# pjookim/srsran-ce-pytorch

Hardware: AMD Instinct MI355X
Metric: slots/sec (273-PRB PUSCH, 4 Rx) (higher is better)
Workload: dtype f32; 1 GPU; pusch273_4rx_filter; n_prb=273, n_sc=3276, n_sym=14, layers=1, rx_ports=4, smoothing=filter, interp=linear, slots_per_gpu=8192, global_slots=8192, rx_layout=[slot][port][sym][sc], parallelism=slot-shard x1, no collective

## Files before the change

srsran_ce_pytorch_amd/csrc/ce_denoise.hip:

```cpp
#include <hip/hip_runtime.h>
#include <stdint.h>
#include <string.h>

#include <type_traits>
#include <vector>

#include "ce_denoise.h"
#include "ce_plan.h"

typedef _Float16 half8 __attribute__((ext_vector_type(8)));
typedef _Float16 half4 __attribute__((ext_vector_type(4)));
typedef _Float16 half2v __attribute__((ext_vector_type(2)));
typedef float f32x4 __attribute__((ext_vector_type(4)));

struct ce_denoiser {
  int device = 0;
  half8* wfrag = nullptr;
  float* bias = nullptr;
};

#ifndef DN_ABLATE
#define DN_ABLATE 0
#endif

namespace {

#ifndef DN_MIN_WAVES
#define DN_MIN_WAVES 3
#endif
#ifndef DN_TWO_BODIES
#define DN_TWO_BODIES 0
#endif
#ifndef DN_L3_BUF
#define DN_L3_BUF 2
#endif
#ifndef DN_T_ROWS
#define DN_T_ROWS 32
#endif
constexpr int DN_T = DN_T_ROWS;
constexpr int DN_NB3 = DN_T / 16;
static_assert(DN_T % 16 == 0, "strip height");
constexpr int DN_NT = 256, DN_COLS = 16, DN_C = CE_DN_CHANNELS;
constexpr int X0_PIX = (DN_T + 6) * DN_COLS + 2;
constexpr int X1_PIX = (DN_T + 5) * DN_COLS + 2;
constexpr int X2_PIX = (DN_T + 2) * DN_COLS + 2;

__device__ __forceinline__ int tap_off(int tap) {
  const int ky = tap / 3, kx = tap - 3 * ky;
  return (ky - 1) * DN_COLS + (kx - 1);
}

constexpr int ROW_BYTES16 = DN_COLS * DN_C * 2;
constexpr int ROW_BYTES0 = DN_COLS * 4;

typedef _Float16 half2x __attribute__((ext_vector_type(2)));
__device__ __forceinline__ float2 masked(float2 v, bool ok) {
  const unsigned m = ok ? 0xFFFFFFFFu : 0u;
  return make_float2(__uint_as_float(__float_as_uint(v.x) & m), __uint_as_float(__float_as_uint(v.y) & m));
}
__device__ __forceinline__ half4 relu_h4(f32x4 acc, unsigned keep) {
  half2x lo = half2x{(_Float16)acc[0], (_Float16)acc[1]}, hi = half2x{(_Float16)acc[2], (_Float16)acc[3]};
  const half2x z = half2x{0, 0}, top = half2x{65504, 65504};
  lo = __builtin_elementwise_min(__builtin_elementwise_max(lo, z), top);
  hi = __builtin_elementwise_min(__builtin_elementwise_max(hi, z), top);
  unsigned ulo, uhi;
  __builtin_memcpy(&ulo, &lo, 4);
  __builtin_memcpy(&uhi, &hi, 4);
  ulo &= keep;
  uhi &= keep;
  __builtin_memcpy(&lo, &ulo, 4);
  __builtin_memcpy(&hi, &uhi, 4);
  return half4{lo[0], lo[1], hi[0], hi[1]};
}

__global__ __launch_bounds__(DN_NT, DN_MIN_WAVES) void ce_denoise_kernel(float2* __restrict__ ch, const half8* __restrict__ wfrag,
                                                            const float* __restrict__ bias, int n_sc, int L) {
  __shared__ __attribute__((aligned(16))) half2v x0[2][X0_PIX];
  __shared__ __attribute__((aligned(16))) _Float16 x1[X1_PIX * DN_C];
  __shared__ __attribute__((aligned(16))) _Float16 x2[X2_PIX * DN_C];
  const int tid = threadIdx.x, lane = tid & 63;
  const int wave = __builtin_amdgcn_readfirstlane(tid >> 6);
  const int n = lane & 15, g = lane >> 4;
  const int64_t plane = blockIdx.x;
  const int64_t item = plane / L;
  const int l = (int)(plane - item * L);
  float2* base = ch + item * (int64_t)n_sc * CE_DN_SYMBOLS * L + l;

  half8 w1 = wfrag[lane], w2[5], w3[9];
#pragma unroll
  for (int m = 0; m < 5; ++m) w2[m] = wfrag[(1 + m) * 64 + lane];
#pragma unroll
  for (int m = 0; m < 9; ++m) w3[m] = wfrag[(6 + m) * 64 + lane];
  f32x4 b1, b2, b3;
#pragma unroll
  for (int i = 0; i < 4; ++i) {
    b1[i] = bias[4 * g + i];
    b2[i] = bias[16 + 4 * g + i];
    b3[i] = g < 2 ? bias[32 + (i & 1)] : 0.f;
  }
  for (int i = tid; i < 2 * X0_PIX; i += DN_NT) (&x0[0][0])[i] = half2v{0, 0};
  for (int i = tid; i < X1_PIX * DN_C; i += DN_NT) x1[i] = 0;
  for (int i = tid; i < X2_PIX * DN_C; i += DN_NT) x2[i] = 0;

  const bool col_ok = n >= 1 && n <= CE_DN_SYMBOLS;
  const unsigned keep = col_ok ? 0xFFFFFFFFu : 0u;
  int rd0[4];
#pragma unroll
  for (int q = 0; q < 4; ++q) {
    const int tap = 4 * g + q;
    rd0[q] = (1 + (wave + 1) * DN_COLS + n + tap_off(tap < 9 ? tap : 4)) * 4;
  }
  constexpr int R2 = (DN_T + 2 + 3) / 4;
  const int a2 = wave * R2 < DN_T + 2 - R2 ? wave * R2 : DN_T + 2 - R2;
  int rdA, rdC, wr2;
  {
    const int pa = 1 + a2 * DN_COLS + n - 1 + (g >> 1), pc = 1 + (a2 + (g >> 1)) * DN_COLS + n + 1, pw = 1 + a2 * DN_COLS + n;
    rdA = pa * (DN_C * 2) + (((g & 1) ^ ((pa >> 2) & 1)) * 16);
    rdC = pc * (DN_C * 2) + (((g & 1) ^ ((pc >> 2) & 1)) * 16);
    wr2 = pw * (DN_C * 2) + ((((g >> 1) & 1) ^ ((pw >> 2) & 1)) * 16) + (g & 1) * 8;
  }
  const int wpix = 1 + wave * DN_COLS + n;
  const int wr = wpix * (DN_C * 2) + ((((g >> 1) & 1) ^ ((wpix >> 2) & 1)) * 16) + (g & 1) * 8;
  constexpr int ST_N = ((DN_T + 6) * DN_COLS + DN_NT - 1) / DN_NT;
  int st_off[ST_N], st_row[ST_N];
  bool st_ok[ST_N];
#pragma unroll
  for (int k = 0; k < ST_N; ++k) {
    const int i = tid + k * DN_NT, sym = (i & 15) - 1;
    st_row[k] = (i >> 4) - 3;
    st_ok[k] = i < (DN_T + 6) * DN_COLS && sym >= 0 && sym < CE_DN_SYMBOLS;
    st_off[k] = (st_row[k] * CE_DN_SYMBOLS + sym) * L;
  }
  int rd3[3];
#pragma unroll
  for (int dx = 0; dx < 3; ++dx) {
    const int pix = 1 + (4 * wave + 3 * (g >> 1)) * DN_COLS + n + dx - 1;
    rd3[dx] = pix * (DN_C * 2) + (((g & 1) ^ ((pix >> 2) & 1)) * 16);
  }
  const int h_row = 4 * wave + 2 * g;
  const int h_off = (h_row * CE_DN_SYMBOLS + (n - 1)) * L;
  const bool h_lane = g < 2 && col_ok;

  float2 st[ST_N];
  auto stage_load = [&](int r0) {
    const float2* sb = base + (int64_t)r0 * CE_DN_SYMBOLS * L;
#pragma unroll
    for (int k = 0; k < ST_N; ++k) {
      const bool ok = st_ok[k] && (unsigned)(r0 + st_row[k]) < (unsigned)n_sc;
      st[k] = masked((DN_ABLATE & 2) ? make_float2(0.f, 0.f) : sb[ok ? st_off[k] : 0], ok);
    }
  };
  auto stage_load_in = [&](int r0) {
    const float2* sb = base + (int64_t)r0 * CE_DN_SYMBOLS * L;
#pragma unroll
    for (int k = 0; k < ST_N; ++k) st[k] = masked((DN_ABLATE & 2) ? make_float2(0.f, 0.f) : sb[st_ok[k] ? st_off[k] : 0], st_ok[k]);
  };
  auto stage_store = [&](int buf) {
#pragma unroll
    for (int k = 0; k < ST_N; ++k) {
      const int i = tid + k * DN_NT;
      if (i < (DN_T + 6) * DN_COLS) x0[buf][1 + i] = half2v{(_Float16)st[k].x, (_Float16)st[k].y};
    }
  };
  stage_load(0);
  __syncthreads();
  stage_store(0);
  __syncthreads();
  const int n_strips = (n_sc + DN_T - 1) / DN_T;
  auto strip = [&](auto edge_tag, int s) __attribute__((always_inline)) {
    constexpr bool EDGE = decltype(edge_tag)::value;
    const int r0 = s * DN_T, buf = s & 1;
    float2* sb = base + (int64_t)r0 * CE_DN_SYMBOLS * L;
    if (s + 1 < n_strips) {
      if (!EDGE && r0 + 2 * DN_T + 3 <= n_sc) stage_load_in(r0 + DN_T); else stage_load(r0 + DN_T);
    }
    float2 hres[DN_NB3][2];
#pragma unroll
    for (int b = 0; b < DN_NB3; ++b)
#pragma unroll
      for (int e = 0; e < 2; ++e) {
        const bool ok = h_lane && (!EDGE || r0 + h_row + 16 * b + e < n_sc);
        hres[b][e] = masked((DN_ABLATE & 2) ? make_float2(0.f, 0.f) : sb[ok ? h_off + (16 * b + e) * CE_DN_SYMBOLS * L : 0], ok);
      }
    {
      const char* xin = reinterpret_cast<const char*>(&x0[buf][0]);
      char* xout = reinterpret_cast<char*>(x1);
      constexpr int NK1 = (DN_T + 4) / 4;
      auto finish1 = [&](f32x4 acc, int k) __attribute__((always_inline)) {
        const int row = r0 - 2 + wave + 4 * k;
        const unsigned rowkeep = (!EDGE || (row >= 0 && row < n_sc)) ? keep : 0u;
        *reinterpret_cast<half4*>(xout + wr + k * 4 * ROW_BYTES16) = relu_h4(acc, rowkeep);
      };
      f32x4 accp = b1;
      half2v px[2][4];
#pragma unroll
      for (int q = 0; q < 4; ++q) px[0][q] = *reinterpret_cast<const half2v*>(xin + rd0[q]);
#pragma unroll
      for (int k = 0; k < NK1; ++k) {
        if (k + 1 < NK1) {
#pragma unroll
          for (int q = 0; q < 4; ++q) px[(k + 1) & 1][q] = *reinterpret_cast<const half2v*>(xin + rd0[q] + (k + 1) * 4 * ROW_BYTES0);
        }
        asm volatile("" ::: "memory");
        half8 b;
#pragma unroll
        for (int q = 0; q < 4; ++q) {
          b[2 * q] = px[k & 1][q][0];
          b[2 * q + 1] = px[k & 1][q][1];
        }
        const f32x4 acc = __builtin_amdgcn_mfma_f32_16x16x32_f16(w1, b, b1, 0, 0, 0);
        if (k > 0) finish1(accp, k - 1);
        accp = acc;
      }
      finish1(accp, NK1 - 1);
    }
    __syncthreads();
    if (s + 1 < n_strips) stage_store(buf ^ 1);
    {
      const char* xin = reinterpret_cast<const char*>(x1);
      char* xout = reinterpret_cast<char*>(x2);
      half8 fa[R2 + 2], fc[R2 + 2];
      auto fetch = [&](int i) __attribute__((always_inline)) {
        fa[i] = *reinterpret_cast<const half8*>(xin + rdA + i * ROW_BYTES16);
        fc[i] = *reinterpret_cast<const half8*>(xin + rdC + i * ROW_BYTES16);
      };
      fetch(0);
      fetch(1);
      fetch(2);
      auto finish2 = [&](f32x4 acc, int j) __attribute__((always_inline)) {
        const int row = r0 - 1 + a2 + j;
        const unsigned rowkeep = (!EDGE || (row >= 0 && row < n_sc)) ? keep : 0u;
        *reinterpret_cast<half4*>(xout + wr2 + j * ROW_BYTES16) = relu_h4(acc, rowkeep);
      };
      f32x4 accp = b2;
#pragma unroll
      for (int j = 0; j < R2; ++j) {
        if (j + 3 < R2 + 2) fetch(j + 3);
        asm volatile("" ::: "memory");
        f32x4 acc = b2;
        acc = __builtin_amdgcn_mfma_f32_16x16x32_f16(w2[0], fa[j], acc, 0, 0, 0);
        acc = __builtin_amdgcn_mfma_f32_16x16x32_f16(w2[1], fa[j + 1], acc, 0, 0, 0);
        acc = __builtin_amdgcn_mfma_f32_16x16x32_f16(w2[2], fa[j + 2], acc, 0, 0, 0);
        acc = __builtin_amdgcn_mfma_f32_16x16x32_f16(w2[3], fc[j], acc, 0, 0, 0);
        acc = __builtin_amdgcn_mfma_f32_16x16x32_f16(w2[4], fc[j + 2], acc, 0, 0, 0);
        if (j > 0) finish2(accp, j - 1);
        accp = acc;
      }
      finish2(accp, R2 - 1);
    }
    __syncthreads();
    {
      const char* xin = reinterpret_cast<const char*>(x2);
      auto finish3 = [&](f32x4 acc, int b) __attribute__((always_inline)) {
#pragma unroll
        for (int e = 0; e < 2; ++e)
          if ((!(DN_ABLATE & 1) || acc[0] == 123.456f) && h_lane && (!EDGE || r0 + h_row + 16 * b + e < n_sc))
            sb[h_off + (16 * b + e) * CE_DN_SYMBOLS * L] = make_float2(hres[b][e].x + acc[2 * e], hres[b][e].y + acc[2 * e + 1]);
      };
      f32x4 accp = b3;
      half8 fr[DN_L3_BUF][9];
#pragma unroll
      for (int j = 0; j < 9; ++j) fr[0][j] = *reinterpret_cast<const half8*>(xin + rd3[j % 3] + (j / 3) * ROW_BYTES16);
#pragma unroll
      for (int b = 0; b < DN_NB3; ++b) {
        if (DN_L3_BUF == 2 && b + 1 < DN_NB3) {
#pragma unroll
          for (int j = 0; j < 9; ++j) fr[(b + 1) & 1][j] = *reinterpret_cast<const half8*>(xin + rd3[j % 3] + (16 * (b + 1) + j / 3) * ROW_BYTES16);
        }
        if (DN_L3_BUF == 1 && b > 0) {
#pragma unroll
          for (int j = 0; j < 9; ++j) fr[0][j] = *reinterpret_cast<const half8*>(xin + rd3[j % 3] + (16 * b + j / 3) * ROW_BYTES16);
        }
        asm volatile("" ::: "memory");
        f32x4 acc = b3;
#pragma unroll
        for (int j = 0; j < 9; ++j) acc = __builtin_amdgcn_mfma_f32_16x16x32_f16(w3[j], fr[b & (DN_L3_BUF - 1)][j], acc, 0, 0, 0);
        if (b > 0) finish3(accp, b - 1);
        accp = acc;
      }
      finish3(accp, DN_NB3 - 1);
    }
  };
#pragma unroll 1
  for (int s = 0; s < n_strips; ++s) {
    const int r0 = s * DN_T;
    if (DN_TWO_BODIES && r0 >= 3 && r0 + DN_T + 3 <= n_sc) strip(std::false_type{}, s);
    else strip(std::true_type{}, s);
  }
}

_Float16 to_h(float v) { return (_Float16)v; }

}

extern "C" int ce_denoiser_create(int32_t device, const float* w1, const float* b1, const float* w2, const float* b2,
                                  const float* w3, const float* b3, ce_denoiser** out) {
  if (!w1 || !b1 || !w2 || !b2 || !w3 || !b3 || !out) return ce_fail(CE_ERR_INVALID, "null argument");
  std::vector<_Float16> frag(15 * 64 * 8, to_h(0.f));
  auto at = [&](int f, int lane, int j) -> _Float16& { return frag[((size_t)f * 64 + lane) * 8 + j]; };
  for (int lane = 0; lane < 64; ++lane) {
    const int co = lane & 15, g = lane >> 4;
    for (int j = 0; j < 8; ++j) {
      const int k = 8 * g + j, tap = k >> 1, ci = k & 1;
      if (tap < 9) at(0, lane, j) = to_h(w1[(co * 2 + ci) * 9 + tap]);
    }
    for (int j = 0; j < 8; ++j) {
      const int ci = 8 * (g & 1) + j, up = g >> 1;
      for (int ky = 0; ky < 3; ++ky) at(1 + ky, lane, j) = to_h(w2[(co * 16 + ci) * 9 + ky * 3 + up]);
      at(4, lane, j) = to_h(w2[(co * 16 + ci) * 9 + up * 3 + 2]);
      if (!up) at(5, lane, j) = to_h(w2[(co * 16 + ci) * 9 + 2 * 3 + 2]);
    }
    if (co < 8)
      for (int m = 0; m < 9; ++m)
        for (int j = 0; j < 8; ++j) {
          const int r = co >> 1, c3 = co & 1, ri = m / 3 + 3 * (g >> 1), dx = m % 3, ci = 8 * (g & 1) + j, ky = ri - r;
          if (ky >= 0 && ky <= 2) at(6 + m, lane, j) = to_h(w3[(c3 * 16 + ci) * 9 + ky * 3 + dx]);
        }
  }
  float bias[48] = {0};
  for (int i = 0; i < 16; ++i) { bias[i] = b1[i]; bias[16 + i] = b2[i]; }
  bias[32] = b3[0];
  bias[33] = b3[1];
  ce_denoiser* d = new ce_denoiser;
  d->device = device;
  CeDeviceScope scope(device);
  hipError_t e = scope.err;
  if (e == hipSuccess) e = hipMalloc(&d->wfrag, frag.size() * sizeof(_Float16));
  if (e == hipSuccess) e = hipMalloc(&d->bias, sizeof(bias));
  if (e == hipSuccess) e = hipMemcpy(d->wfrag, frag.data(), frag.size() * sizeof(_Float16), hipMemcpyHostToDevice);
  if (e == hipSuccess) e = hipMemcpy(d->bias, bias, sizeof(bias), hipMemcpyHostToDevice);
  if (e != hipSuccess) {
    ce_denoiser_destroy(d);
    return ce_fail(CE_ERR_HIP, "denoiser upload: %s", hipGetErrorString(e));
  }
  *out = d;
  return CE_OK;
}

extern "C" void ce_denoiser_destroy(ce_denoiser* d) {
  if (!d) return;
  if (d->wfrag) (void)hipFree(d->wfrag);
  if (d->bias) (void)hipFree(d->bias);
  delete d;
}

extern "C" int ce_denoise_batch(const ce_denoiser* d, void* ch_est, int64_t n_items, int32_t n_sc, int32_t n_sym,
                                int32_t n_layers, void* stream) {
  if (!d || (!ch_est && n_items > 0)) return ce_fail(CE_ERR_INVALID, "null argument");
  if (n_sym != CE_DN_SYMBOLS) return ce_fail(CE_ERR_UNSUPPORTED, "the denoiser is built for 14-symbol grids (got %d)", n_sym);
  if (n_items < 0 || n_sc < 1 || n_layers < 1 || n_layers > CE_MAX_LAYERS) return ce_fail(CE_ERR_INVALID, "bad shape");
  const int64_t planes = n_items * n_layers;
  if (planes == 0) return CE_OK;
  if (planes > 0x7FFFFFFFll) return ce_fail(CE_ERR_UNSUPPORTED, "%lld planes in one launch", (long long)planes);
  CeDeviceScope scope(d->device);
  if (scope.err != hipSuccess) return ce_fail(CE_ERR_HIP, "device %d: %s", d->device, hipGetErrorString(scope.err));
  hipLaunchKernelGGL(ce_denoise_kernel, dim3((unsigned)planes), dim3(DN_NT), 0, (hipStream_t)stream,
                     reinterpret_cast<float2*>(ch_est), d->wfrag, d->bias, n_sc, n_layers);
  const hipError_t e = hipGetLastError();
  return e == hipSuccess ? CE_OK : ce_fail(CE_ERR_HIP, "denoise launch: %s", hipGetErrorString(e));
}
```

Baseline: 3.648 million slots/s.

## Cut address arithmetic and register pressure in denoiser strip loop

Replaces the per-element int64 offset arithmetic with precomputed 32-bit byte offsets, plus a single out-of-range sentinel offset, for the staging and residual loads. The staging buffer now lives inside each strip, and the last-iteration store guard is simplified using a static half-wave layout. The layer-3 fragment double-buffer is dropped in favour of direct LDS reads feeding each MFMA. The interior/edge two-body specialisation is turned on by default. The aim is fewer VGPRs and fewer scalar/vector address instructions, in exchange for less explicit load latency hiding in layer 3 and a larger code size.

```diff
diff --git a/srsran_ce_pytorch_amd/csrc/ce_denoise.hip b/srsran_ce_pytorch_amd/csrc/ce_denoise.hip
--- a/srsran_ce_pytorch_amd/csrc/ce_denoise.hip
+++ b/srsran_ce_pytorch_amd/csrc/ce_denoise.hip
@@ -29,10 +29,7 @@
 #define DN_MIN_WAVES 3
 #endif
 #ifndef DN_TWO_BODIES
-#define DN_TWO_BODIES 0
-#endif
-#ifndef DN_L3_BUF
-#define DN_L3_BUF 2
+#define DN_TWO_BODIES 1
 #endif
 #ifndef DN_T_ROWS
 #define DN_T_ROWS 32
@@ -122,14 +119,15 @@
   const int wpix = 1 + wave * DN_COLS + n;
   const int wr = wpix * (DN_C * 2) + ((((g >> 1) & 1) ^ ((wpix >> 2) & 1)) * 16) + (g & 1) * 8;
   constexpr int ST_N = ((DN_T + 6) * DN_COLS + DN_NT - 1) / DN_NT;
-  int st_off[ST_N], st_row[ST_N];
+  const unsigned st_none = 3u * CE_DN_SYMBOLS * L * 8u;
+  const int st_row0 = (tid >> 4) - 3;
+  unsigned st_byte[ST_N];
   bool st_ok[ST_N];
 #pragma unroll
   for (int k = 0; k < ST_N; ++k) {
     const int i = tid + k * DN_NT, sym = (i & 15) - 1;
-    st_row[k] = (i >> 4) - 3;
     st_ok[k] = i < (DN_T + 6) * DN_COLS && sym >= 0 && sym < CE_DN_SYMBOLS;
-    st_off[k] = (st_row[k] * CE_DN_SYMBOLS + sym) * L;
+    st_byte[k] = st_ok[k] ? (unsigned)(((i >> 4) * CE_DN_SYMBOLS + sym) * L) * 8u : st_none;
   }
   int rd3[3];
 #pragma unroll
@@ -138,50 +136,63 @@
     rd3[dx] = pix * (DN_C * 2) + (((g & 1) ^ ((pix >> 2) & 1)) * 16);
   }
   const int h_row = 4 * wave + 2 * g;
-  const int h_off = (h_row * CE_DN_SYMBOLS + (n - 1)) * L;
-  const bool h_lane = g < 2 && col_ok;
-
-  float2 st[ST_N];
-  auto stage_load = [&](int r0) {
-    const float2* sb = base + (int64_t)r0 * CE_DN_SYMBOLS * L;
+  int h_flag = g < 2 && col_ok;
+  asm volatile("" : "+v"(h_flag));
+  const bool h_lane = h_flag != 0;
+  const unsigned h_byte = h_lane ? (unsigned)((h_row * CE_DN_SYMBOLS + (n - 1)) * L) * 8u : 0u;
+
+  const char* basec = reinterpret_cast<const char*>(base);
+  auto strip_byte = [&](int row) { return (unsigned)(row * CE_DN_SYMBOLS * L) * 8u; };
+  auto stage_load = [&](float2 (&st)[ST_N], int r0) {
 #pragma unroll
     for (int k = 0; k < ST_N; ++k) {
-      const bool ok = st_ok[k] && (unsigned)(r0 + st_row[k]) < (unsigned)n_sc;
-      st[k] = masked((DN_ABLATE & 2) ? make_float2(0.f, 0.f) : sb[ok ? st_off[k] : 0], ok);
+      const bool in_grid = (unsigned)(r0 + st_row0 + 16 * k) < (unsigned)n_sc;
+      const unsigned off = strip_byte(r0 - 3) + (in_grid ? st_byte[k] : st_none);
+      st[k] = masked((DN_ABLATE & 2) ? make_float2(0.f, 0.f) : *reinterpret_cast<const float2*>(basec + off), st_ok[k] & in_grid);
     }
   };
-  auto stage_load_in = [&](int r0) {
-    const float2* sb = base + (int64_t)r0 * CE_DN_SYMBOLS * L;
-#pragma unroll
-    for (int k = 0; k < ST_N; ++k) st[k] = masked((DN_ABLATE & 2) ? make_float2(0.f, 0.f) : sb[st_ok[k] ? st_off[k] : 0], st_ok[k]);
+  auto stage_load_in = [&](float2 (&st)[ST_N], int r0) {
+#pragma unroll
+    for (int k = 0; k < ST_N; ++k)
+      st[k] = masked((DN_ABLATE & 2) ? make_float2(0.f, 0.f) : *reinterpret_cast<const float2*>(basec + (strip_byte(r0 - 3) + st_byte[k])), st_ok[k]);
   };
-  auto stage_store = [&](int buf) {
+  constexpr int ST_PIX = (DN_T + 6) * DN_COLS;
+  static_assert(ST_PIX % DN_NT % 64 == 32, "the left-over half wave");
+  const int st_last = tid + (ST_N - 1) * DN_NT < ST_PIX ? 1 + tid + (ST_N - 1) * DN_NT : 1 + (tid + (ST_N - 1) * DN_NT - ST_PIX) * DN_COLS;
+  auto stage_store = [&](const float2 (&st)[ST_N], int buf) {
 #pragma unroll
     for (int k = 0; k < ST_N; ++k) {
-      const int i = tid + k * DN_NT;
-      if (i < (DN_T + 6) * DN_COLS) x0[buf][1 + i] = half2v{(_Float16)st[k].x, (_Float16)st[k].y};
+      const half2v v = half2v{(_Float16)st[k].x, (_Float16)st[k].y};
+      if (k < ST_N - 1) x0[buf][1 + tid + k * DN_NT] = v;
+      else if (wave * 64 + k * DN_NT < ST_PIX) x0[buf][st_last] = v;
     }
   };
-  stage_load(0);
-  __syncthreads();
-  stage_store(0);
+  {
+    float2 st[ST_N];
+    stage_load(st, 0);
+    __syncthreads();
+    stage_store(st, 0);
+  }
   __syncthreads();
   const int n_strips = (n_sc + DN_T - 1) / DN_T;
   auto strip = [&](auto edge_tag, int s) __attribute__((always_inline)) {
     constexpr bool EDGE = decltype(edge_tag)::value;
     const int r0 = s * DN_T, buf = s & 1;
-    float2* sb = base + (int64_t)r0 * CE_DN_SYMBOLS * L;
+    float2 st[ST_N] = {};
     if (s + 1 < n_strips) {
-      if (!EDGE && r0 + 2 * DN_T + 3 <= n_sc) stage_load_in(r0 + DN_T); else stage_load(r0 + DN_T);
+      if (!EDGE && r0 + 2 * DN_T + 3 <= n_sc) stage_load_in(st, r0 + DN_T); else stage_load(st, r0 + DN_T);
     }
     float2 hres[DN_NB3][2];
+    const unsigned h_cur = strip_byte(r0) + h_byte;
+    auto h_ptr = [&](int b, int e) __attribute__((always_inline)) {
+      const unsigned row_byte = strip_byte(16 * b + e);
+      if (!EDGE) return const_cast<char*>(basec) + (size_t)row_byte + h_cur;
+      return const_cast<char*>(basec) + (r0 + h_row + 16 * b + e < n_sc ? row_byte + h_cur : strip_byte(r0));
+    };
 #pragma unroll
     for (int b = 0; b < DN_NB3; ++b)
 #pragma unroll
-      for (int e = 0; e < 2; ++e) {
-        const bool ok = h_lane && (!EDGE || r0 + h_row + 16 * b + e < n_sc);
-        hres[b][e] = masked((DN_ABLATE & 2) ? make_float2(0.f, 0.f) : sb[ok ? h_off + (16 * b + e) * CE_DN_SYMBOLS * L : 0], ok);
-      }
+      for (int e = 0; e < 2; ++e) hres[b][e] = (DN_ABLATE & 2) ? make_float2(0.f, 0.f) : *reinterpret_cast<const float2*>(h_ptr(b, e));
     {
       const char* xin = reinterpret_cast<const char*>(&x0[buf][0]);
       char* xout = reinterpret_cast<char*>(x1);
@@ -215,7 +226,7 @@
       finish1(accp, NK1 - 1);
     }
     __syncthreads();
-    if (s + 1 < n_strips) stage_store(buf ^ 1);
+    if (s + 1 < n_strips) stage_store(st, buf ^ 1);
     {
       const char* xin = reinterpret_cast<const char*>(x1);
       char* xout = reinterpret_cast<char*>(x2);
@@ -252,29 +263,22 @@
     {
       const char* xin = reinterpret_cast<const char*>(x2);
       auto finish3 = [&](f32x4 acc, int b) __attribute__((always_inline)) {
-#pragma unroll
-        for (int e = 0; e < 2; ++e)
-          if ((!(DN_ABLATE & 1) || acc[0] == 123.456f) && h_lane && (!EDGE || r0 + h_row + 16 * b + e < n_sc))
-            sb[h_off + (16 * b + e) * CE_DN_SYMBOLS * L] = make_float2(hres[b][e].x + acc[2 * e], hres[b][e].y + acc[2 * e + 1]);
+        if (h_lane) {
+#pragma unroll
+          for (int e = 0; e < 2; ++e)
+            if ((!(DN_ABLATE & 1) || acc[0] == 123.456f) && (!EDGE || r0 + h_row + 16 * b + e < n_sc))
+              *reinterpret_cast<float2*>(h_ptr(b, e)) = make_float2(hres[b][e].x + acc[2 * e], hres[b][e].y + acc[2 * e + 1]);
+        }
+      };
+      auto frag3 = [&](int b, int j) __attribute__((always_inline)) {
+        return *reinterpret_cast<const half8*>(xin + rd3[j % 3] + (16 * b + j / 3) * ROW_BYTES16);
       };
       f32x4 accp = b3;
-      half8 fr[DN_L3_BUF][9];
-#pragma unroll
-      for (int j = 0; j < 9; ++j) fr[0][j] = *reinterpret_cast<const half8*>(xin + rd3[j % 3] + (j / 3) * ROW_BYTES16);
 #pragma unroll
       for (int b = 0; b < DN_NB3; ++b) {
-        if (DN_L3_BUF == 2 && b + 1 < DN_NB3) {
-#pragma unroll
-          for (int j = 0; j < 9; ++j) fr[(b + 1) & 1][j] = *reinterpret_cast<const half8*>(xin + rd3[j % 3] + (16 * (b + 1) + j / 3) * ROW_BYTES16);
-        }
-        if (DN_L3_BUF == 1 && b > 0) {
-#pragma unroll
-          for (int j = 0; j < 9; ++j) fr[0][j] = *reinterpret_cast<const half8*>(xin + rd3[j % 3] + (16 * b + j / 3) * ROW_BYTES16);
-        }
-        asm volatile("" ::: "memory");
         f32x4 acc = b3;
 #pragma unroll
-        for (int j = 0; j < 9; ++j) acc = __builtin_amdgcn_mfma_f32_16x16x32_f16(w3[j], fr[b & (DN_L3_BUF - 1)][j], acc, 0, 0, 0);
+        for (int j = 0; j < 9; ++j) acc = __builtin_amdgcn_mfma_f32_16x16x32_f16(w3[j], frag3(b, j), acc, 0, 0, 0);
         if (b > 0) finish3(accp, b - 1);
         accp = acc;
       }
```

New measurement: 3.597 million slots/s. 0.986x the previous value.

## Replace LDS-staged denoiser with register-resident row streaming using DPP neighbor exchange

Applied to the files above, without the earlier changes.

Rewrites the 3-layer conv denoiser so each wave streams its own band of subcarrier rows. Intermediate activations stay in registers, and horizontal neighbours are exchanged with DPP row shifts instead of going through shared memory. This removes all LDS buffers and per-strip block barriers. Weight fragments are repacked for the new lane layout, and layer 3 now produces 8-row blocks with more MFMAs per block. The trade-offs are higher register pressure (min waves lowered to 2) and a sequential dependency along each wave's band, with halo rows recomputed at band boundaries.

```diff
diff --git a/srsran_ce_pytorch_amd/csrc/ce_denoise.hip b/srsran_ce_pytorch_amd/csrc/ce_denoise.hip
--- a/srsran_ce_pytorch_amd/csrc/ce_denoise.hip
+++ b/srsran_ce_pytorch_amd/csrc/ce_denoise.hip
@@ -10,8 +10,24 @@
 
 typedef _Float16 half8 __attribute__((ext_vector_type(8)));
 typedef _Float16 half4 __attribute__((ext_vector_type(4)));
-typedef _Float16 half2v __attribute__((ext_vector_type(2)));
 typedef float f32x4 __attribute__((ext_vector_type(4)));
+typedef unsigned u32x4 __attribute__((ext_vector_type(4)));
+
+#ifndef DN_ABLATE
+#define DN_ABLATE 0
+#endif
+#ifndef DN_L3_ROWS
+#define DN_L3_ROWS 8
+#endif
+#ifndef DN_MIN_WAVES
+#define DN_MIN_WAVES 2
+#endif
+
+constexpr int DN_BH = DN_L3_ROWS;
+constexpr int DN_P = (DN_BH + 2) / 2;
+constexpr int DN_K3 = 3 * DN_P;
+constexpr int DN_NFRAG = 1 + 5 + DN_K3;
+static_assert(DN_BH == 4 || DN_BH == 8, "layer-3 block height");
 
 struct ce_denoiser {
   int device = 0;
@@ -19,65 +35,46 @@
   float* bias = nullptr;
 };
 
-#ifndef DN_ABLATE
-#define DN_ABLATE 0
-#endif
-
 namespace {
 
-#ifndef DN_MIN_WAVES
-#define DN_MIN_WAVES 3
-#endif
-#ifndef DN_TWO_BODIES
-#define DN_TWO_BODIES 0
-#endif
-#ifndef DN_L3_BUF
-#define DN_L3_BUF 2
-#endif
-#ifndef DN_T_ROWS
-#define DN_T_ROWS 32
-#endif
-constexpr int DN_T = DN_T_ROWS;
-constexpr int DN_NB3 = DN_T / 16;
-static_assert(DN_T % 16 == 0, "strip height");
-constexpr int DN_NT = 256, DN_COLS = 16, DN_C = CE_DN_CHANNELS;
-constexpr int X0_PIX = (DN_T + 6) * DN_COLS + 2;
-constexpr int X1_PIX = (DN_T + 5) * DN_COLS + 2;
-constexpr int X2_PIX = (DN_T + 2) * DN_COLS + 2;
-
-__device__ __forceinline__ int tap_off(int tap) {
-  const int ky = tap / 3, kx = tap - 3 * ky;
-  return (ky - 1) * DN_COLS + (kx - 1);
-}
-
-constexpr int ROW_BYTES16 = DN_COLS * DN_C * 2;
-constexpr int ROW_BYTES0 = DN_COLS * 4;
+constexpr int DN_NT = 256;
 
 typedef _Float16 half2x __attribute__((ext_vector_type(2)));
-__device__ __forceinline__ float2 masked(float2 v, bool ok) {
-  const unsigned m = ok ? 0xFFFFFFFFu : 0u;
-  return make_float2(__uint_as_float(__float_as_uint(v.x) & m), __uint_as_float(__float_as_uint(v.y) & m));
-}
-__device__ __forceinline__ half4 relu_h4(f32x4 acc, unsigned keep) {
+constexpr unsigned DN_TOP = 0x7BFF7BFFu;
+__device__ __forceinline__ half4 relu_h4(f32x4 acc, unsigned top_bits) {
   half2x lo = half2x{(_Float16)acc[0], (_Float16)acc[1]}, hi = half2x{(_Float16)acc[2], (_Float16)acc[3]};
-  const half2x z = half2x{0, 0}, top = half2x{65504, 65504};
+  const half2x z = half2x{0, 0}, top = __builtin_bit_cast(half2x, top_bits);
   lo = __builtin_elementwise_min(__builtin_elementwise_max(lo, z), top);
   hi = __builtin_elementwise_min(__builtin_elementwise_max(hi, z), top);
-  unsigned ulo, uhi;
-  __builtin_memcpy(&ulo, &lo, 4);
-  __builtin_memcpy(&uhi, &hi, 4);
-  ulo &= keep;
-  uhi &= keep;
-  __builtin_memcpy(&lo, &ulo, 4);
-  __builtin_memcpy(&hi, &uhi, 4);
   return half4{lo[0], lo[1], hi[0], hi[1]};
 }
 
-__global__ __launch_bounds__(DN_NT, DN_MIN_WAVES) void ce_denoise_kernel(float2* __restrict__ ch, const half8* __restrict__ wfrag,
+__device__ __forceinline__ unsigned from_left(unsigned v) {
+  return (unsigned)__builtin_amdgcn_update_dpp(0, (int)v, 0x111, 0xF, 0xF, true);
+}
+__device__ __forceinline__ unsigned from_right(unsigned v) {
+  return (unsigned)__builtin_amdgcn_update_dpp(0, (int)v, 0x101, 0xF, 0xF, true);
+}
+
+struct Piece { unsigned a, b; };
+struct Row { Piece p[3]; };
+
+__device__ __forceinline__ half8 frag(unsigned a, unsigned b, unsigned c, unsigned d) {
+  return __builtin_bit_cast(half8, u32x4{a, b, c, d});
+}
+__device__ __forceinline__ half8 frag(Piece x, Piece y) { return frag(x.a, x.b, y.a, y.b); }
+
+__device__ __forceinline__ Row make_row(f32x4 acc, unsigned top) {
+  const half4 h = relu_h4(acc, top);
+  Row r;
+  __builtin_memcpy(&r.p[1], &h, 8);
+  r.p[0] = Piece{from_left(r.p[1].a), from_left(r.p[1].b)};
+  r.p[2] = Piece{from_right(r.p[1].a), from_right(r.p[1].b)};
+  return r;
+}
+
+__global__ __launch_bounds__(DN_NT, DN_MIN_WAVES) void ce_denoise_kernel(float2* ch, const half8* __restrict__ wfrag,
                                                             const float* __restrict__ bias, int n_sc, int L) {
-  __shared__ __attribute__((aligned(16))) half2v x0[2][X0_PIX];
-  __shared__ __attribute__((aligned(16))) _Float16 x1[X1_PIX * DN_C];
-  __shared__ __attribute__((aligned(16))) _Float16 x2[X2_PIX * DN_C];
   const int tid = threadIdx.x, lane = tid & 63;
   const int wave = __builtin_amdgcn_readfirstlane(tid >> 6);
   const int n = lane & 15, g = lane >> 4;
@@ -86,206 +83,161 @@
   const int l = (int)(plane - item * L);
   float2* base = ch + item * (int64_t)n_sc * CE_DN_SYMBOLS * L + l;
 
-  half8 w1 = wfrag[lane], w2[5], w3[9];
+  half8 w1 = wfrag[lane], w2[5], w3[DN_K3];
 #pragma unroll
   for (int m = 0; m < 5; ++m) w2[m] = wfrag[(1 + m) * 64 + lane];
 #pragma unroll
-  for (int m = 0; m < 9; ++m) w3[m] = wfrag[(6 + m) * 64 + lane];
+  for (int m = 0; m < DN_K3; ++m) w3[m] = wfrag[(6 + m) * 64 + lane];
   f32x4 b1, b2, b3;
 #pragma unroll
   for (int i = 0; i < 4; ++i) {
     b1[i] = bias[4 * g + i];
     b2[i] = bias[16 + 4 * g + i];
-    b3[i] = g < 2 ? bias[32 + (i & 1)] : 0.f;
-  }
-  for (int i = tid; i < 2 * X0_PIX; i += DN_NT) (&x0[0][0])[i] = half2v{0, 0};
-  for (int i = tid; i < X1_PIX * DN_C; i += DN_NT) x1[i] = 0;
-  for (int i = tid; i < X2_PIX * DN_C; i += DN_NT) x2[i] = 0;
-
-  const bool col_ok = n >= 1 && n <= CE_DN_SYMBOLS;
-  const unsigned keep = col_ok ? 0xFFFFFFFFu : 0u;
-  int rd0[4];
-#pragma unroll
-  for (int q = 0; q < 4; ++q) {
-    const int tap = 4 * g + q;
-    rd0[q] = (1 + (wave + 1) * DN_COLS + n + tap_off(tap < 9 ? tap : 4)) * 4;
-  }
-  constexpr int R2 = (DN_T + 2 + 3) / 4;
-  const int a2 = wave * R2 < DN_T + 2 - R2 ? wave * R2 : DN_T + 2 - R2;
-  int rdA, rdC, wr2;
-  {
-    const int pa = 1 + a2 * DN_COLS + n - 1 + (g >> 1), pc = 1 + (a2 + (g >> 1)) * DN_COLS + n + 1, pw = 1 + a2 * DN_COLS + n;
-    rdA = pa * (DN_C * 2) + (((g & 1) ^ ((pa >> 2) & 1)) * 16);
-    rdC = pc * (DN_C * 2) + (((g & 1) ^ ((pc >> 2) & 1)) * 16);
-    wr2 = pw * (DN_C * 2) + ((((g >> 1) & 1) ^ ((pw >> 2) & 1)) * 16) + (g & 1) * 8;
-  }
-  const int wpix = 1 + wave * DN_COLS + n;
-  const int wr = wpix * (DN_C * 2) + ((((g >> 1) & 1) ^ ((wpix >> 2) & 1)) * 16) + (g & 1) * 8;
-  constexpr int ST_N = ((DN_T + 6) * DN_COLS + DN_NT - 1) / DN_NT;
-  int st_off[ST_N], st_row[ST_N];
-  bool st_ok[ST_N];
-#pragma unroll
-  for (int k = 0; k < ST_N; ++k) {
-    const int i = tid + k * DN_NT, sym = (i & 15) - 1;
-    st_row[k] = (i >> 4) - 3;
-    st_ok[k] = i < (DN_T + 6) * DN_COLS && sym >= 0 && sym < CE_DN_SYMBOLS;
-    st_off[k] = (st_row[k] * CE_DN_SYMBOLS + sym) * L;
-  }
-  int rd3[3];
-#pragma unroll
-  for (int dx = 0; dx < 3; ++dx) {
-    const int pix = 1 + (4 * wave + 3 * (g >> 1)) * DN_COLS + n + dx - 1;
-    rd3[dx] = pix * (DN_C * 2) + (((g & 1) ^ ((pix >> 2) & 1)) * 16);
-  }
-  const int h_row = 4 * wave + 2 * g;
-  const int h_off = (h_row * CE_DN_SYMBOLS + (n - 1)) * L;
-  const bool h_lane = g < 2 && col_ok;
-
-  float2 st[ST_N];
-  auto stage_load = [&](int r0) {
-    const float2* sb = base + (int64_t)r0 * CE_DN_SYMBOLS * L;
-#pragma unroll
-    for (int k = 0; k < ST_N; ++k) {
-      const bool ok = st_ok[k] && (unsigned)(r0 + st_row[k]) < (unsigned)n_sc;
-      st[k] = masked((DN_ABLATE & 2) ? make_float2(0.f, 0.f) : sb[ok ? st_off[k] : 0], ok);
-    }
-  };
-  auto stage_load_in = [&](int r0) {
-    const float2* sb = base + (int64_t)r0 * CE_DN_SYMBOLS * L;
-#pragma unroll
-    for (int k = 0; k < ST_N; ++k) st[k] = masked((DN_ABLATE & 2) ? make_float2(0.f, 0.f) : sb[st_ok[k] ? st_off[k] : 0], st_ok[k]);
-  };
-  auto stage_store = [&](int buf) {
-#pragma unroll
-    for (int k = 0; k < ST_N; ++k) {
-      const int i = tid + k * DN_NT;
-      if (i < (DN_T + 6) * DN_COLS) x0[buf][1 + i] = half2v{(_Float16)st[k].x, (_Float16)st[k].y};
-    }
-  };
-  stage_load(0);
+    b3[i] = 2 * g < DN_BH ? bias[32 + (i & 1)] : 0.f;
+  }
+
+  const int n_blk = (n_sc + DN_BH - 1) / DN_BH, band = ((n_blk + 3) / 4) * DN_BH;
+  const int r_lo = wave * band;
+  const int r_hi = r_lo + band < n_sc ? r_lo + band : n_sc;
+  const int nb = r_lo < n_sc ? (r_hi - r_lo + DN_BH - 1) / DN_BH : 0;
+
+  const int S = CE_DN_SYMBOLS * L;
+  const bool col_ok = n < CE_DN_SYMBOLS;
+  const unsigned top = col_ok ? DN_TOP : 0u;
+  const int nc = col_ok ? n : CE_DN_SYMBOLS - 1;
+  const unsigned t_keep = (col_ok && g < 3) ? 0xFFFFFFFFu : 0u;
+  const int t_dg = (col_ok && g < 3) ? g - 1 : -0x40000000;
+  const int t_off = ((g < 3 ? g : 2) * CE_DN_SYMBOLS + nc) * L;
+  const bool h_lane = col_ok && 2 * g < DN_BH;
+  const int h_row = h_lane ? 2 * g : 0x40000000;
+  const int h_off = ((2 * g < DN_BH ? 2 * g : 0) * CE_DN_SYMBOLS + nc) * L;
+
+  auto tile_load = [&](auto edge_tag, int u) __attribute__((always_inline)) -> float2 {
+    if (DN_ABLATE & 2) return make_float2(0.f, 0.f);
+    if constexpr (decltype(edge_tag)::value) {
+      const bool ok = (unsigned)(u + t_dg) < (unsigned)n_sc;
+      return base[ok ? (u - 1) * S + t_off : 0];
+    } else {
+      return (base + (int64_t)(u - 1) * S)[t_off];
+    }
+  };
+  auto tile_cvt = [&](auto edge_tag, float2 v, int u) __attribute__((always_inline)) -> unsigned {
+    const half2x h = half2x{(_Float16)v.x, (_Float16)v.y};
+    unsigned d;
+    __builtin_memcpy(&d, &h, 4);
+    if constexpr (decltype(edge_tag)::value) return (unsigned)(u + t_dg) < (unsigned)n_sc ? d : 0u;
+    else return d & t_keep;
+  };
+  auto res_load = [&](auto edge_tag, int o0, int e) __attribute__((always_inline)) -> float2 {
+    if (DN_ABLATE & 2) return make_float2(0.f, 0.f);
+    if constexpr (decltype(edge_tag)::value) {
+      const bool ok = o0 + e + h_row < n_sc;
+      return base[ok ? (o0 + e) * S + h_off : 0];
+    } else {
+      return (base + (int64_t)(o0 + e) * S)[h_off];
+    }
+  };
+  auto row_top = [&](auto edge_tag, int u) __attribute__((always_inline)) -> unsigned {
+    if constexpr (decltype(edge_tag)::value) return (unsigned)u < (unsigned)n_sc ? top : 0u;
+    else return top;
+  };
+  auto layer1 = [&](unsigned d) __attribute__((always_inline)) -> f32x4 {
+    return __builtin_amdgcn_mfma_f32_16x16x32_f16(w1, frag(from_left(d), d, from_right(d), 0u), b1, 0, 0, 0);
+  };
+  auto layer2 = [&](const Row& y0, const Row& y1, const Row& y2) __attribute__((always_inline)) -> f32x4 {
+    f32x4 acc = b2;
+    acc = __builtin_amdgcn_mfma_f32_16x16x32_f16(w2[0], frag(y0.p[0], y0.p[1]), acc, 0, 0, 0);
+    acc = __builtin_amdgcn_mfma_f32_16x16x32_f16(w2[1], frag(y1.p[0], y1.p[1]), acc, 0, 0, 0);
+    acc = __builtin_amdgcn_mfma_f32_16x16x32_f16(w2[3], frag(y0.p[2], y1.p[2]), acc, 0, 0, 0);
+    acc = __builtin_amdgcn_mfma_f32_16x16x32_f16(w2[2], frag(y2.p[0], y2.p[1]), acc, 0, 0, 0);
+    acc = __builtin_amdgcn_mfma_f32_16x16x32_f16(w2[4], frag(y2.p[2].a, y2.p[2].b, 0u, 0u), acc, 0, 0, 0);
+    return acc;
+  };
+
+  const std::true_type edge{};
+  const std::false_type inner{};
+  Row ya{}, yb{}, xa{}, xb{};
+  unsigned d[DN_BH];
+  unsigned saved[3] = {0u, 0u, 0u};
+#pragma unroll
+  for (int k = 0; k < DN_BH; ++k) d[k] = 0u;
+
+  if (nb > 0) {
+    const int u_s = r_lo + nb * DN_BH - 1;
+    float2 ts[3], tp[4], T[DN_BH];
+#pragma unroll
+    for (int j = 0; j < 3; ++j) ts[j] = tile_load(edge, u_s + j);
+#pragma unroll
+    for (int j = 0; j < 4; ++j) tp[j] = tile_load(edge, r_lo - 2 + j);
+#pragma unroll
+    for (int k = 0; k < DN_BH; ++k) T[k] = tile_load(edge, r_lo + 2 + k);
+#pragma unroll
+    for (int j = 0; j < 3; ++j) saved[j] = tile_cvt(edge, ts[j], u_s + j);
+    Row y[4];
+#pragma unroll
+    for (int j = 0; j < 4; ++j) y[j] = make_row(layer1(tile_cvt(edge, tp[j], r_lo - 2 + j)), row_top(edge, r_lo - 2 + j));
+    xa = make_row(layer2(y[0], y[1], y[2]), row_top(edge, r_lo - 1));
+    xb = make_row(layer2(y[1], y[2], y[3]), row_top(edge, r_lo));
+    ya = y[2];
+    yb = y[3];
+#pragma unroll
+    for (int k = 0; k < DN_BH; ++k) d[k] = tile_cvt(edge, T[k], r_lo + 2 + k);
+  }
   __syncthreads();
-  stage_store(0);
-  __syncthreads();
-  const int n_strips = (n_sc + DN_T - 1) / DN_T;
-  auto strip = [&](auto edge_tag, int s) __attribute__((always_inline)) {
+  __builtin_amdgcn_s_waitcnt(0);
+
+  auto block = [&](auto edge_tag, int o0, bool last) __attribute__((always_inline)) {
     constexpr bool EDGE = decltype(edge_tag)::value;
-    const int r0 = s * DN_T, buf = s & 1;
-    float2* sb = base + (int64_t)r0 * CE_DN_SYMBOLS * L;
-    if (s + 1 < n_strips) {
-      if (!EDGE && r0 + 2 * DN_T + 3 <= n_sc) stage_load_in(r0 + DN_T); else stage_load(r0 + DN_T);
-    }
-    float2 hres[DN_NB3][2];
-#pragma unroll
-    for (int b = 0; b < DN_NB3; ++b)
-#pragma unroll
-      for (int e = 0; e < 2; ++e) {
-        const bool ok = h_lane && (!EDGE || r0 + h_row + 16 * b + e < n_sc);
-        hres[b][e] = masked((DN_ABLATE & 2) ? make_float2(0.f, 0.f) : sb[ok ? h_off + (16 * b + e) * CE_DN_SYMBOLS * L : 0], ok);
-      }
-    {
-      const char* xin = reinterpret_cast<const char*>(&x0[buf][0]);
-      char* xout = reinterpret_cast<char*>(x1);
-      constexpr int NK1 = (DN_T + 4) / 4;
-      auto finish1 = [&](f32x4 acc, int k) __attribute__((always_inline)) {
-        const int row = r0 - 2 + wave + 4 * k;
-        const unsigned rowkeep = (!EDGE || (row >= 0 && row < n_sc)) ? keep : 0u;
-        *reinterpret_cast<half4*>(xout + wr + k * 4 * ROW_BYTES16) = relu_h4(acc, rowkeep);
-      };
-      f32x4 accp = b1;
-      half2v px[2][4];
-#pragma unroll
-      for (int q = 0; q < 4; ++q) px[0][q] = *reinterpret_cast<const half2v*>(xin + rd0[q]);
-#pragma unroll
-      for (int k = 0; k < NK1; ++k) {
-        if (k + 1 < NK1) {
-#pragma unroll
-          for (int q = 0; q < 4; ++q) px[(k + 1) & 1][q] = *reinterpret_cast<const half2v*>(xin + rd0[q] + (k + 1) * 4 * ROW_BYTES0);
-        }
-        asm volatile("" ::: "memory");
-        half8 b;
-#pragma unroll
-        for (int q = 0; q < 4; ++q) {
-          b[2 * q] = px[k & 1][q][0];
-          b[2 * q + 1] = px[k & 1][q][1];
-        }
-        const f32x4 acc = __builtin_amdgcn_mfma_f32_16x16x32_f16(w1, b, b1, 0, 0, 0);
-        if (k > 0) finish1(accp, k - 1);
-        accp = acc;
-      }
-      finish1(accp, NK1 - 1);
-    }
-    __syncthreads();
-    if (s + 1 < n_strips) stage_store(buf ^ 1);
-    {
-      const char* xin = reinterpret_cast<const char*>(x1);
-      char* xout = reinterpret_cast<char*>(x2);
-      half8 fa[R2 + 2], fc[R2 + 2];
-      auto fetch = [&](int i) __attribute__((always_inline)) {
-        fa[i] = *reinterpret_cast<const half8*>(xin + rdA + i * ROW_BYTES16);
-        fc[i] = *reinterpret_cast<const half8*>(xin + rdC + i * ROW_BYTES16);
-      };
-      fetch(0);
-      fetch(1);
-      fetch(2);
-      auto finish2 = [&](f32x4 acc, int j) __attribute__((always_inline)) {
-        const int row = r0 - 1 + a2 + j;
-        const unsigned rowkeep = (!EDGE || (row >= 0 && row < n_sc)) ? keep : 0u;
-        *reinterpret_cast<half4*>(xout + wr2 + j * ROW_BYTES16) = relu_h4(acc, rowkeep);
-      };
-      f32x4 accp = b2;
-#pragma unroll
-      for (int j = 0; j < R2; ++j) {
-        if (j + 3 < R2 + 2) fetch(j + 3);
-        asm volatile("" ::: "memory");
-        f32x4 acc = b2;
-        acc = __builtin_amdgcn_mfma_f32_16x16x32_f16(w2[0], fa[j], acc, 0, 0, 0);
-        acc = __builtin_amdgcn_mfma_f32_16x16x32_f16(w2[1], fa[j + 1], acc, 0, 0, 0);
-        acc = __builtin_amdgcn_mfma_f32_16x16x32_f16(w2[2], fa[j + 2], acc, 0, 0, 0);
-        acc = __builtin_amdgcn_mfma_f32_16x16x32_f16(w2[3], fc[j], acc, 0, 0, 0);
-        acc = __builtin_amdgcn_mfma_f32_16x16x32_f16(w2[4], fc[j + 2], acc, 0, 0, 0);
-        if (j > 0) finish2(accp, j - 1);
-        accp = acc;
-      }
-      finish2(accp, R2 - 1);
-    }
-    __syncthreads();
-    {
-      const char* xin = reinterpret_cast<const char*>(x2);
-      auto finish3 = [&](f32x4 acc, int b) __attribute__((always_inline)) {
-#pragma unroll
-        for (int e = 0; e < 2; ++e)
-          if ((!(DN_ABLATE & 1) || acc[0] == 123.456f) && h_lane && (!EDGE || r0 + h_row + 16 * b + e < n_sc))
-            sb[h_off + (16 * b + e) * CE_DN_SYMBOLS * L] = make_float2(hres[b][e].x + acc[2 * e], hres[b][e].y + acc[2 * e + 1]);
-      };
-      f32x4 accp = b3;
-      half8 fr[DN_L3_BUF][9];
-#pragma unroll
-      for (int j = 0; j < 9; ++j) fr[0][j] = *reinterpret_cast<const half8*>(xin + rd3[j % 3] + (j / 3) * ROW_BYTES16);
-#pragma unroll
-      for (int b = 0; b < DN_NB3; ++b) {
-        if (DN_L3_BUF == 2 && b + 1 < DN_NB3) {
-#pragma unroll
-          for (int j = 0; j < 9; ++j) fr[(b + 1) & 1][j] = *reinterpret_cast<const half8*>(xin + rd3[j % 3] + (16 * (b + 1) + j / 3) * ROW_BYTES16);
-        }
-        if (DN_L3_BUF == 1 && b > 0) {
-#pragma unroll
-          for (int j = 0; j < 9; ++j) fr[0][j] = *reinterpret_cast<const half8*>(xin + rd3[j % 3] + (16 * b + j / 3) * ROW_BYTES16);
-        }
-        asm volatile("" ::: "memory");
-        f32x4 acc = b3;
-#pragma unroll
-        for (int j = 0; j < 9; ++j) acc = __builtin_amdgcn_mfma_f32_16x16x32_f16(w3[j], fr[b & (DN_L3_BUF - 1)][j], acc, 0, 0, 0);
-        if (b > 0) finish3(accp, b - 1);
-        accp = acc;
-      }
-      finish3(accp, DN_NB3 - 1);
-    }
+    float2 cr[2], T[DN_BH];
+#pragma unroll
+    for (int e = 0; e < 2; ++e) cr[e] = res_load(edge_tag, o0, e);
+#pragma unroll
+    for (int k = 0; k < DN_BH; ++k) T[k] = tile_load(edge_tag, o0 + DN_BH + 2 + k);
+    asm volatile("" : "+v"(d[0]) : : "memory");
+#pragma unroll
+    for (int j = 0; j < 3; ++j) d[DN_BH - 3 + j] = last ? saved[j] : d[DN_BH - 3 + j];
+    f32x4 a1[DN_BH];
+#pragma unroll
+    for (int k = 0; k < DN_BH; ++k) a1[k] = layer1(d[k]);
+    Row y[DN_BH + 2], z[DN_BH + 2];
+    y[0] = ya;
+    y[1] = yb;
+    z[0] = xa;
+    z[1] = xb;
+    f32x4 accp = b2;
+#pragma unroll
+    for (int k = 0; k < DN_BH; ++k) {
+      y[2 + k] = make_row(a1[k], row_top(edge_tag, o0 + 2 + k));
+      const f32x4 acc = layer2(y[k], y[k + 1], y[k + 2]);
+      if (k > 0) z[1 + k] = make_row(accp, row_top(edge_tag, o0 + k));
+      accp = acc;
+    }
+    z[DN_BH + 1] = make_row(accp, row_top(edge_tag, o0 + DN_BH));
+    f32x4 acc = b3;
+#pragma unroll
+    for (int ri = 0; ri < DN_P; ++ri)
+#pragma unroll
+      for (int s = 0; s < 3; ++s)
+        acc = __builtin_amdgcn_mfma_f32_16x16x32_f16(w3[3 * ri + s], frag(z[ri].p[s], z[ri + DN_P].p[s]), acc, 0, 0, 0);
+#pragma unroll
+    for (int k = 0; k < DN_BH; ++k) d[k] = tile_cvt(edge_tag, T[k], o0 + DN_BH + 2 + k);
+    asm volatile("" : "+v"(d[0]) : : "memory");
+#pragma unroll
+    for (int e = 0; e < 2; ++e) {
+      const bool ok = EDGE ? o0 + e + h_row < n_sc : h_lane;
+      if ((!(DN_ABLATE & 1) || acc[0] == 123.456f) && ok)
+        (base + (int64_t)(o0 + e) * S)[h_off] = make_float2(cr[e].x + acc[2 * e], cr[e].y + acc[2 * e + 1]);
+    }
+    ya = y[DN_BH];
+    yb = y[DN_BH + 1];
+    xa = z[DN_BH];
+    xb = z[DN_BH + 1];
   };
 #pragma unroll 1
-  for (int s = 0; s < n_strips; ++s) {
-    const int r0 = s * DN_T;
-    if (DN_TWO_BODIES && r0 >= 3 && r0 + DN_T + 3 <= n_sc) strip(std::false_type{}, s);
-    else strip(std::true_type{}, s);
+  for (int b = 0; b < nb; ++b) {
+    const int o0 = r_lo + b * DN_BH;
+    if (o0 >= 3 && o0 + 2 * DN_BH + 3 <= n_sc) block(inner, o0, b == nb - 1);
+    else block(edge, o0, b == nb - 1);
   }
 }
 
@@ -296,26 +248,26 @@
 extern "C" int ce_denoiser_create(int32_t device, const float* w1, const float* b1, const float* w2, const float* b2,
                                   const float* w3, const float* b3, ce_denoiser** out) {
   if (!w1 || !b1 || !w2 || !b2 || !w3 || !b3 || !out) return ce_fail(CE_ERR_INVALID, "null argument");
-  std::vector<_Float16> frag(15 * 64 * 8, to_h(0.f));
+  std::vector<_Float16> frag(DN_NFRAG * 64 * 8, to_h(0.f));
   auto at = [&](int f, int lane, int j) -> _Float16& { return frag[((size_t)f * 64 + lane) * 8 + j]; };
   for (int lane = 0; lane < 64; ++lane) {
     const int co = lane & 15, g = lane >> 4;
     for (int j = 0; j < 8; ++j) {
-      const int k = 8 * g + j, tap = k >> 1, ci = k & 1;
-      if (tap < 9) at(0, lane, j) = to_h(w1[(co * 2 + ci) * 9 + tap]);
+      const int q = j >> 1, c = j & 1;
+      if (g < 3 && q < 3) at(0, lane, j) = to_h(w1[(co * 2 + c) * 9 + g * 3 + q]);
     }
     for (int j = 0; j < 8; ++j) {
-      const int ci = 8 * (g & 1) + j, up = g >> 1;
-      for (int ky = 0; ky < 3; ++ky) at(1 + ky, lane, j) = to_h(w2[(co * 16 + ci) * 9 + ky * 3 + up]);
-      at(4, lane, j) = to_h(w2[(co * 16 + ci) * 9 + up * 3 + 2]);
-      if (!up) at(5, lane, j) = to_h(w2[(co * 16 + ci) * 9 + 2 * 3 + 2]);
-    }
-    if (co < 8)
-      for (int m = 0; m < 9; ++m)
-        for (int j = 0; j < 8; ++j) {
-          const int r = co >> 1, c3 = co & 1, ri = m / 3 + 3 * (g >> 1), dx = m % 3, ci = 8 * (g & 1) + j, ky = ri - r;
-          if (ky >= 0 && ky <= 2) at(6 + m, lane, j) = to_h(w3[(c3 * 16 + ci) * 9 + ky * 3 + dx]);
+      const int p = j >> 2, ci = 4 * g + (j & 3);
+      for (int ky = 0; ky < 3; ++ky) at(1 + ky, lane, j) = to_h(w2[(co * 16 + ci) * 9 + ky * 3 + p]);
+      at(4, lane, j) = to_h(w2[(co * 16 + ci) * 9 + p * 3 + 2]);
+      if (p == 0) at(5, lane, j) = to_h(w2[(co * 16 + ci) * 9 + 2 * 3 + 2]);
+      const int r = co >> 1, c3 = co & 1;
+      if (r < DN_BH)
+        for (int m = 0; m < DN_K3; ++m) {
+          const int ri = m / 3, s = m % 3, ky = ri + DN_P * p - r;
+          if (ky >= 0 && ky <= 2) at(6 + m, lane, j) = to_h(w3[(c3 * 16 + ci) * 9 + ky * 3 + s]);
         }
+    }
   }
   float bias[48] = {0};
   for (int i = 0; i < 16; ++i) { bias[i] = b1[i]; bias[16 + i] = b2[i]; }
```

Result: no change. 3.592 million slots/s before, 3.570 million slots/s after (-0.6%).
